# Ham3798/shielded-pool-pinocchio-solana

Hardware: AMD Instinct MI355X
Metric: Groth16 proofs/sec (higher is better)
Workload: dtype u32x8 (254-bit Montgomery integers); 1 GPU; audit_circuit (RLWE, const-PK; scripts/generate_audit.py:246-465), batch of 2048 independent proofs per GPU per step, every row a distinct witness; circuit=audit, n_constraints=29178, n_wires=35432, domain=32768, batch_per_gpu=2048, n_distinct_witnesses=2048, table_bytes=226725433344, parallelism=independent proofs x1, pk_bytes=9850060

## Files before the change

### include/spp.h

```cpp
#ifndef SPP_H
#define SPP_H
#include <stddef.h>
#include <stdint.h>
#ifdef __cplusplus
extern "C" {
#endif

#define SPP_OK 0
#define SPP_ERR_BAD_INPUT (-1)
#define SPP_ERR_NO_DEVICE (-2)
#define SPP_ERR_IO (-3)
#define SPP_ERR_UNSAT (-4)
#define SPP_ERR_HIP (-5)
#define SPP_ERR_NOT_IMPLEMENTED (-6)
#define SPP_ERR_FORMAT (-7)

#define SPP_CIRCUIT_WITHDRAW 1
#define SPP_CIRCUIT_AUDIT 2
#define SPP_CIRCUIT_WITHDRAW_REFSHAPE 3
#define SPP_CIRCUIT_WITHDRAW_DEPTH20 4

#define SPP_PROOF_LEN 388
#define SPP_WITHDRAW_PW_LEN 172
#define SPP_AUDIT_PW_LEN 76
// ... 36 lines not shown
int spp_circuit_msm_windows(const spp_circuit* c, uint32_t bits[7]);
int spp_circuit_msm_table_rows(const spp_circuit* c, uint32_t rows[7]);
int spp_circuit_small_rows(const spp_circuit* c, uint32_t out[2]);
uint64_t spp_circuit_table_bytes(const spp_circuit* c);

int spp_prove_batch(spp_circuit* c, size_t count, const uint8_t* inputs, const uint8_t* rs, uint8_t* proofs, uint8_t* pws,
                    int32_t* status);
int spp_prove_batch_device(spp_circuit* c, size_t count, const void* d_inputs, const void* d_rs, void* d_proofs, void* d_pws,
                           void* d_status);
int spp_sync(spp_circuit* c);
int spp_commitment_challenge(spp_circuit* c, size_t count, const uint8_t* inputs, uint8_t* challenges);
int spp_last_timings(spp_circuit* c, float ms[9]);
int spp_timings(spp_circuit* c, int which, float ms[9]);

int spp_msm_kernel_ms(spp_circuit* c, int which, float ms[7]);
int spp_set_serial(spp_circuit* c, int on);

int spp_prove_withdraw(spp_circuit* c, const spp_withdraw_inputs* in, const uint8_t rs_seed[64], uint8_t proof[SPP_PROOF_LEN],
                       uint8_t pw[SPP_WITHDRAW_PW_LEN]);

int spp_verify(const uint8_t* vk, size_t vk_len, const uint8_t* proof, size_t proof_len, const uint8_t* pw, size_t pw_len, int* ok);

int spp_debug_witness(spp_circuit* c, uint8_t* out, size_t n_wires);

#define SPP_ARITH_FR 0x000u
#define SPP_ARITH_FQ 0x100u
int spp_debug_arith(spp_ctx* ctx, uint32_t selector, uint32_t arg, size_t n, const uint32_t* in, size_t in_words, uint32_t* out,
                    size_t out_words);

int spp_rlwe_witness_batch(spp_ctx* ctx, const uint32_t* pk_a, const uint32_t* pk_b, size_t count, const int8_t* r, const int8_t* e1,
                           const int8_t* e2, const uint8_t* msg, uint32_t* c0, uint32_t* c1, int32_t* k0, int32_t* k1,
                           uint8_t* packed_be);
int spp_rlwe_witness_batch_device(spp_ctx* ctx, const void* d_pk_a, const void* d_pk_b, size_t count, const void* d_r, const void* d_e1,
                                  const void* d_e2, const void* d_msg, void* d_c0, void* d_c1, void* d_k0, void* d_k1,
                                  void* d_packed_be);
int spp_ctx_sync(spp_ctx* ctx);
int spp_poseidon_hash_batch(spp_ctx* ctx, size_t count, int arity, const uint8_t* in, uint8_t* out);
int spp_merkle_root_batch(spp_ctx* ctx, size_t count, uint32_t depth, const uint8_t* leaves, const uint64_t* indices,
                          const uint8_t* siblings, uint8_t* roots);
int spp_merkle_build(spp_ctx* ctx, size_t n_leaves, uint32_t depth, const uint8_t* leaves, size_t n_queries,
                     const uint64_t* query_indices, uint8_t* siblings_out, uint8_t* root_out);
typedef struct spp_merkle_tree spp_merkle_tree;
int spp_merkle_tree_new(spp_ctx* ctx, uint32_t depth, spp_merkle_tree** out);
void spp_merkle_tree_free(spp_merkle_tree* t);
uint64_t spp_merkle_tree_size(const spp_merkle_tree* t);
int spp_merkle_tree_insert(spp_merkle_tree* t, size_t count, const uint8_t* leaves, uint64_t* first_index);
// ... 121 lines not shown
```

### shielded-pool-pinocchio-solana_amd/csrc/kernels.hpp

```cpp
#pragma once
#include <hip/hip_runtime.h>
#include <stdint.h>
#include "bn254.hpp"
#include "f29.hpp"
#include "msm_plan.hpp"
#include "msm_ragged.hpp"
#include "rlwe_ntt.hpp"

namespace spp {

struct DevSparse {
  const uint32_t* rowptr;
  const uint32_t* wire;
  const uint32_t* coeff;
  const uint32_t* lit;
};
static constexpr uint32_t COEFF_ONE = 0x80000000u;
static constexpr uint32_t COEFF_MINUS_ONE = 0x40000000u;
static constexpr uint32_t COEFF_MASK = 0x3fffffffu;

struct HashConsts {
  const Fr* pos3_rc;  const Fr* pos3_mds;
  const Fr* pos5_rc;  const Fr* pos5_mds;
  const Fr* p2_rc;    const Fr* p2_mu;
// ... 115 lines not shown
                       int32_t* ok, uint32_t* list, uint32_t* n_list, uint32_t* stats);
void launch_verify_rlc_list(hipStream_t st, const VerifyKeyDev* vk, const RlcKeyDev* rk, const uint8_t* proofs, const uint8_t* pws, uint32_t pw_len,
                            uint32_t max_count, const uint32_t* in_list, const uint32_t* n_in, const RlcSeed& seed, uint32_t group, W256* ws,
                            uint32_t* live, int32_t* ok, uint32_t* list, uint32_t* n_list, uint32_t* stats);
struct PoolSet;
struct PoolState;
void launch_pool_screen_audit(hipStream_t st, const PoolSet& audits, uint64_t salt, const uint8_t* pws, uint32_t count, int32_t* prov, uint32_t* list,
                              uint32_t* n_list);
void launch_pool_screen_withdraw(hipStream_t st, const PoolState* state, const PoolSet& audits, const PoolSet& nullifiers, uint64_t salt,
                                 const uint8_t* pws, const uint8_t* recipients, uint32_t count, int32_t* prov, uint64_t* amounts, uint32_t* list,
                                 uint32_t* n_list);
struct PoolLogView;
void launch_pool_screen_withdraw_log(hipStream_t st, const PoolLogView& view, const PoolSet& audits, const PoolSet& nullifiers, uint64_t salt,
                                     const uint8_t* pws, const uint8_t* recipients, const uint32_t* deposits_before, const uint32_t* audits_before,
                                     uint32_t count, int32_t* prov, uint64_t* amounts, uint32_t* list, uint32_t* n_list);
void launch_pool_scatter(hipStream_t st, const uint32_t* pos, uint32_t count, const int32_t* codes, int32_t* result, const uint64_t* amounts,
                         uint64_t* amounts_out);
void launch_pool_screen_import(hipStream_t st, const PoolSet& set, uint64_t salt, const uint8_t* keys, uint32_t count, int32_t* prov);
void launch_pool_contains(hipStream_t st, const PoolSet& set, uint64_t salt, const uint8_t* keys, uint32_t count, uint8_t* present);
void launch_pool_resolve(hipStream_t st, uint32_t* slots, uint32_t mask, uint64_t salt, const uint8_t* keys, uint32_t stride, uint32_t count,
                         const int32_t* prov, const int32_t* proof_ok, int32_t dup, int32_t* result);
void launch_pool_commit(hipStream_t st, const PoolSet& set, uint64_t salt, const uint8_t* keys, uint32_t stride, uint32_t count, const int32_t* result,
                        uint32_t* set_count);
void launch_spmv_check(hipStream_t st, DevCircuit dc, const Fr* W, Fr* abc, uint32_t n, uint32_t P, uint32_t* status, int16_t* small = nullptr);

void launch_ntt(hipStream_t st, Fr* data, uint32_t logn, uint32_t P, const Fr* tw, bool dif, uint32_t nbatch, size_t batch_stride,
                const Fr* post = nullptr);
void launch_scale_rows(hipStream_t st, Fr* data, const Fr* table, uint32_t n, uint32_t P, uint32_t nbatch, size_t batch_stride);
void launch_qap_pointwise(hipStream_t st, Fr* abc, uint32_t n, uint32_t P, Fr zinv);
void launch_qap_product(hipStream_t st, Fr* abc, uint32_t n, uint32_t P);

template <class F>
struct MsmWalk;
template <>
struct MsmWalk<Fq> {
  static constexpr uint32_t waves_per_simd = 3;
  static constexpr uint32_t rows_waves_per_simd = 2;
  static constexpr bool gather_ahead = false;
  static constexpr int product_form = F29_SCAN_SERIAL;
  static constexpr uint32_t occ(uint32_t Wt) { return Wt == 1 ? waves_per_simd : rows_waves_per_simd; }
};
template <>
struct MsmWalk<Fq2> {
  static constexpr uint32_t waves_per_simd = 2;
  static constexpr uint32_t rows_waves_per_simd = 1;
  static constexpr bool gather_ahead = false;
  static constexpr int product_form = F29_COLUMNS;
  static constexpr uint32_t occ(uint32_t Wt) { return Wt == 1 ? waves_per_simd : rows_waves_per_simd; }
};
template <class F>
void launch_build_table(hipStream_t st, const Affine<F>* bases, uint32_t N, uint32_t c, uint32_t Wt, uint32_t row0, uint32_t nrows,
                        Affine<F>* table, XYZZ<F>* tmp, F* tmp_pre, const MsmBlock* blocks = nullptr, uint32_t E = 0);
void launch_msm_digits(hipStream_t st, const uint32_t* rows, const Fr* scalars, int16_t* dig, uint32_t N, uint32_t P, uint32_t c);
template <class F>
void launch_msm_accumulate(hipStream_t st, const Affine<F>* table, const MsmBlock* blocks, const int16_t* dig, XYZZ<F>* partial, uint32_t N, uint32_t P,
                           uint32_t c, const MsmPlan& pl, hipEvent_t ev_start = nullptr, hipEvent_t ev_stop = nullptr, uint32_t* redo_count = nullptr);
template <class F>
void launch_msm_reduce(hipStream_t st, XYZZ<F>* partial, XYZZ<F>* out, uint32_t P, const MsmPlan& pl, uint32_t c, bool empty);
static constexpr uint32_t MSM_FOLD_SETS = 8;
static constexpr uint32_t MSM_FOLD_RADIX = 8;
template <class F>
struct MsmFoldSets {
  XYZZ<F>* partial[MSM_FOLD_SETS];
  XYZZ<F>* out[MSM_FOLD_SETS];
  uint32_t Sg[MSM_FOLD_SETS], R[MSM_FOLD_SETS], c[MSM_FOLD_SETS];
  uint32_t cur[MSM_FOLD_SETS], half[MSM_FOLD_SETS];
};
template <class F>
void launch_msm_reduce_multi(hipStream_t st, MsmFoldSets<F> fs, uint32_t nsets, uint32_t P);

void launch_g1_eval_basis(hipStream_t st, const G1Affine* pts, uint32_t n_pts, uint32_t logn, const Fr* scale, const Fr* tw_inv, G1XYZZ* work,
                          G1Affine* out);

void launch_g1_column_sums(hipStream_t st, const G1Affine* base, const uint32_t* row, const Fr* coeff, uint32_t nterms, const uint32_t* seg,
                           uint32_t nseg, G1XYZZ* work, G1Affine* out);

// ... 31 lines not shown
```

### shielded-pool-pinocchio-solana_amd/csrc/kernels_msm.hip

```cpp
#include "msm_table.hpp"

namespace spp {

template void launch_build_table<Fq>(hipStream_t, const Affine<Fq>*, uint32_t, uint32_t, uint32_t, uint32_t, uint32_t, Affine<Fq>*,
                                     XYZZ<Fq>*, Fq*, const MsmBlock*, uint32_t);
template void launch_msm_accumulate<Fq>(hipStream_t, const Affine<Fq>*, const MsmBlock*, const int16_t*, XYZZ<Fq>*, uint32_t, uint32_t, uint32_t,
                                        const MsmPlan&, hipEvent_t, hipEvent_t, uint32_t*);
template void launch_msm_reduce_multi<Fq>(hipStream_t, MsmFoldSets<Fq>, uint32_t, uint32_t);
template void launch_msm_reduce<Fq>(hipStream_t, XYZZ<Fq>*, XYZZ<Fq>*, uint32_t, const MsmPlan&, uint32_t, bool);
template void launch_fixed_base_mul<Fq>(hipStream_t, const Affine<Fq>*, uint32_t, const Fr*, uint32_t, Affine<Fq>*);

__global__ void __launch_bounds__(256) k_msm_digits(const uint32_t* __restrict__ rows, const Fr* __restrict__ scalars,
                                                    int16_t* __restrict__ dig, uint32_t N, uint32_t P, uint32_t Pp, uint32_t c, uint32_t W) {
  const uint64_t g = (uint64_t)blockIdx.x * blockDim.x + threadIdx.x;
  const uint32_t p = (uint32_t)(g % Pp), i = (uint32_t)(g / Pp);
  if (i >= N || p >= P) return;
  const Fr s = scalars[(size_t)rows[i] * P + p];
  uint32_t l[8];
  s.to_canonical(l);
  const bool neg = canonical_gt_half<FrParams>(l);
  if (neg) {
    uint32_t t[8];
    canonical_negate<FrParams>(l, t);
    SPP_UNROLL for (int k = 0; k < 8; k++) l[k] = t[k];
  }
  const uint32_t mask = (1u << c) - 1u, half = 1u << (c - 1);
  uint32_t carry = 0;
  int16_t* out = dig + (size_t)i * Pp + p;
  const size_t plane = (size_t)N * Pp;
#pragma unroll 1
  for (uint32_t j = 0; j < W; j++) {
    const uint32_t d = (l[0] & mask) + carry;
    SPP_UNROLL for (int k = 0; k < 7; k++) l[k] = (l[k] >> c) | (l[k + 1] << (32 - c));
    l[7] >>= c;
    const bool over = neg ? d > half : d >= half;
    int v = over ? (int)d - (int)(1u << c) : (int)d;
    carry = over ? 1u : 0u;
    if (neg) v = -v;
    out[(size_t)j * plane] = (int16_t)v;
  }
}
void launch_msm_digits(hipStream_t st, const uint32_t* rows, const Fr* scalars, int16_t* dig, uint32_t N, uint32_t P, uint32_t c) {
  if (N == 0 || P == 0) return;
  const uint32_t Pp = msm_padded_batch(P);
  const uint64_t lanes = (uint64_t)N * Pp;
  hipLaunchKernelGGL(k_msm_digits, dim3((uint32_t)((lanes + 255) / 256)), dim3(256), 0, st, rows, scalars, dig, N, P, Pp, c, msm_windows(c));
}

__device__ __forceinline__ XYZZ<Fq> g1_scalar_mul(const XYZZ<Fq>& pt, const Fr& k) {
  uint32_t c[8];
  k.to_canonical(c);
  XYZZ<Fq> acc = XYZZ<Fq>::infinity();
  if (pt.is_inf()) return acc;
#pragma unroll 1
  for (int w = 7; w >= 0; w--) {
    const uint32_t word = w == 0 ? c[0] : w == 1 ? c[1] : w == 2 ? c[2] : w == 3 ? c[3] : w == 4 ? c[4] : w == 5 ? c[5] : w == 6 ? c[6] : c[7];
#pragma unroll 1
    for (int bit = 31; bit >= 0; bit--) {
      acc.dbl_inplace();
      if ((word >> bit) & 1) acc.add(pt);
    }
  }
  return acc;
}
__global__ void __launch_bounds__(64) k_g1_dft_load(const G1Affine* __restrict__ pts, uint32_t n_pts, const Fr* __restrict__ scale,
                                                    G1XYZZ* __restrict__ x, uint32_t n) {
  const uint32_t j = blockIdx.x * blockDim.x + threadIdx.x;
  if (j >= n) return;
  x[j] = j < n_pts ? g1_scalar_mul(G1XYZZ::from_affine(pts[j]), scale[j]) : G1XYZZ::infinity();
// ... 51 lines not shown
```

### shielded-pool-pinocchio-solana_amd/csrc/kernels_solve.hip

```cpp
#include "kernels.hpp"
#include "circuit.hpp"
#include "poseidon29.hpp"
#include "poseidon2.hpp"
#include "gnark_hints.hpp"
#include "sha256.hpp"

namespace spp {

__device__ __forceinline__ Fr dev_row_dot(const DevSparse& m, const Fr* __restrict__ coeffs, uint32_t k, uint32_t k_end_skip,
                                           const Fr* __restrict__ W, uint32_t P, uint32_t p, uint32_t first = 0, uint32_t step = 1) {
  Fr acc = Fr::zero();
  const uint32_t b = m.rowptr[k] + first, e = m.rowptr[k + 1] - k_end_skip;
  for (uint32_t t = b; t < e; t += step) {
    const uint32_t ci = m.coeff[t];
    Fr w = W[(size_t)m.wire[t] * P + p];
    if (ci & COEFF_ONE) acc = acc + w;
    else if (ci & COEFF_MINUS_ONE) acc = acc - w;
    else acc = acc + coeffs[ci & COEFF_MASK] * w;
  }
  return acc;
}

__global__ void __launch_bounds__(256) k_load_inputs(const uint8_t* __restrict__ in_be, const uint8_t* __restrict__ rs_be,
                                                     Fr* __restrict__ W, uint32_t n_inputs, uint32_t n_wires, uint32_t P) {
// ... 754 lines not shown
  int v = pos ? (int)c[0] : neg ? -(int)n[0] : 0;
  const int lo = dc.sm_lo[s];
  if ((!pos && !neg) || v < lo || v > lo + 255) {
    atomicOr(&status[p], 1u);
    v = 0;
  }
  small[g] = (int16_t)v;
}
__global__ void __launch_bounds__(256) k_spmv_small_rows(DevCircuit dc, const int16_t* __restrict__ small, const Fr* __restrict__ W,
                                                         Fr* __restrict__ abc, uint32_t n, uint32_t P) {
  const uint64_t g = (uint64_t)blockIdx.x * blockDim.x + threadIdx.x;
  if (g >= (uint64_t)dc.sm_nrows * P) return;
  const uint32_t p = (uint32_t)(g % P), r = (uint32_t)(g / P);
  const uint32_t b = dc.sm_rowptr[r], e = dc.sm_rowptr[r + 1];
  long long acc = 0;
  for (uint32_t t = b; t < e; t++) acc += (long long)dc.sm_coef[t] * (long long)small[(size_t)dc.sm_slot[t] * P + p];
  const uint32_t ro = dc.sm_row_out[r], mat = ro >> 30, k = ro & 0x3fffffffu;
  const Fr mag = Fr::from_u64((uint64_t)(acc < 0 ? -acc : acc));
  Fr v = acc < 0 ? mag.neg() : mag;
  for (uint32_t t = dc.sm_rest_ptr[r]; t < dc.sm_rest_ptr[r + 1]; t++) v = v + dc.coeffs[dc.sm_rest_coeff[t]] * W[(size_t)dc.sm_rest_wire[t] * P + p];
  abc[(size_t)mat * n * P + (size_t)k * P + p] = v;
}

__global__ void __launch_bounds__(256) k_spmv_check(DevCircuit dc, const Fr* __restrict__ W, Fr* __restrict__ abc, uint32_t n, uint32_t P,
                                                    uint32_t* __restrict__ status) {
  const uint64_t g = (uint64_t)blockIdx.x * blockDim.x + threadIdx.x;
  const uint64_t lanes = (uint64_t)(dc.n_runs + (n - dc.n_constraints)) * P;
  if (g >= lanes) return;
  const uint32_t p = (uint32_t)(g % P), r = (uint32_t)(g / P);
  const uint64_t total = (uint64_t)n * P;
  if (r >= dc.n_runs) {
    const uint64_t o = (uint64_t)(dc.n_constraints + (r - dc.n_runs)) * P + p;
    abc[o] = Fr::zero();
    abc[total + o] = Fr::zero();
    abc[2 * total + o] = Fr::zero();
    return;
  }
  const uint32_t k0 = dc.run_start[r], k1 = dc.run_start[r + 1];
  const uint8_t* __restrict__ rs = dc.row_small;
  const Fr b = (rs && (rs[k0] & 2)) ? abc[total + (uint64_t)k0 * P + p] : dev_row_dot_wide(dc.B, dc.coeffs, k0, W, P, p);
  bool bad = false;
  for (uint32_t k = k0; k < k1; k++) {
    const uint64_t o = (uint64_t)k * P + p;
    const uint32_t f = rs ? rs[k] : 0u;
    const Fr a = (f & 1) ? abc[o] : dev_row_dot_wide(dc.A, dc.coeffs, k, W, P, p);
    const Fr c = (f & 4) ? abc[2 * total + o] : dev_row_dot_wide(dc.C, dc.coeffs, k, W, P, p);
    bad |= (a * b != c);
    abc[o] = a;
    abc[total + o] = b;
    abc[2 * total + o] = c;
  }
  if (bad) atomicOr(&status[p], 1u);
}
static constexpr uint32_t LONG_G = 16;
__global__ void __launch_bounds__(1024) k_spmv_long_rows(DevCircuit dc, const Fr* __restrict__ W, Fr* __restrict__ abc, uint32_t n, uint32_t P) {
  __shared__ Fr part[LONG_G][64];
  const uint32_t lane = threadIdx.x & 63, sub = threadIdx.x >> 6, p = blockIdx.x * 64 + lane;
  const uint32_t code = dc.lg_rows[blockIdx.y], mi = code >> 30, k = code & 0x3fffffffu;
  const DevSparse& m = mi == 0 ? dc.A : mi == 1 ? dc.B : dc.C;
  part[sub][lane] = p < P ? dev_row_dot_wide(m, dc.coeffs, k, W, P, p, sub, LONG_G) : Fr::zero();
  __syncthreads();
  if (sub != 0 || p >= P) return;
  Fr acc = part[0][lane];
  SPP_UNROLL for (uint32_t q = 1; q < LONG_G; q++) acc = acc + part[q][lane];
  abc[(uint64_t)mi * n * P + (uint64_t)k * P + p] = acc;
}

static constexpr uint32_t SPMV_G = 16;
__device__ __forceinline__ Fr group_sum(Fr v) {
  SPP_UNROLL for (uint32_t off = SPMV_G / 2; off >= 1; off >>= 1) {
    Fr o;
    SPP_UNROLL for (int i = 0; i < 8; i++) o.l[i] = __shfl_xor(v.l[i], off);
    v = v + o;
  }
  return v;
}
__global__ void __launch_bounds__(256) k_spmv_check_rows(DevCircuit dc, const Fr* __restrict__ W, Fr* __restrict__ abc, uint32_t n, uint32_t P,
                                                         uint32_t* __restrict__ status) {
  const uint64_t g = (uint64_t)blockIdx.x * blockDim.x + threadIdx.x;
  const uint64_t total = (uint64_t)n * P;
  const uint64_t e = g / SPMV_G;
  const uint32_t sub = (uint32_t)(g % SPMV_G);
  const bool live = e < total;
  const uint32_t p = live ? (uint32_t)(e % P) : 0, k = live ? (uint32_t)(e / P) : dc.n_constraints;
  Fr a = Fr::zero(), b = Fr::zero(), c = Fr::zero();
  if (k < dc.n_constraints) {
    a = dev_row_dot_wide(dc.A, dc.coeffs, k, W, P, p, sub, SPMV_G);
    b = dev_row_dot_wide(dc.B, dc.coeffs, k, W, P, p, sub, SPMV_G);
    c = dev_row_dot_wide(dc.C, dc.coeffs, k, W, P, p, sub, SPMV_G);
  }
  a = group_sum(a);
  b = group_sum(b);
  c = group_sum(c);
  if (!live || sub != 0) return;
  if (a * b != c) atomicOr(&status[p], 1u);
  abc[e] = a;
  abc[total + e] = b;
  abc[2 * total + e] = c;
}
void launch_spmv_check(hipStream_t st, DevCircuit dc, const Fr* W, Fr* abc, uint32_t n, uint32_t P, uint32_t* status, int16_t* small) {
  if ((uint64_t)dc.n_runs * P < 65536 || (P <= 64 && dc.max_row_terms > 1024)) {
    const uint64_t lanes = (uint64_t)n * P * SPMV_G;
    hipLaunchKernelGGL(k_spmv_check_rows, dim3((uint32_t)((lanes + 255) / 256)), dim3(256), 0, st, dc, W, abc, n, P, status);
    return;
  }
  if (small && dc.sm_nrows) {
    const uint64_t l1 = (uint64_t)dc.sm_nslots * P, l2 = (uint64_t)dc.sm_nrows * P;
    hipLaunchKernelGGL(k_small_extract, dim3((uint32_t)((l1 + 255) / 256)), dim3(256), 0, st, dc, W, small, P, status);
    hipLaunchKernelGGL(k_spmv_small_rows, dim3((uint32_t)((l2 + 255) / 256)), dim3(256), 0, st, dc, small, W, abc, n, P);
  } else {
    dc.row_small = dc.row_long;
  }
  if (dc.lg_n) hipLaunchKernelGGL(k_spmv_long_rows, dim3((P + 63) / 64, dc.lg_n), dim3(1024), 0, st, dc, W, abc, n, P);
  const uint64_t lanes = (uint64_t)(dc.n_runs + (n - dc.n_constraints)) * P;
  hipLaunchKernelGGL(k_spmv_check, dim3((uint32_t)((lanes + 255) / 256)), dim3(256), 0, st, dc, W, abc, n, P, status);
}

}
```

### shielded-pool-pinocchio-solana_amd/csrc/spp_circuit.hpp

```cpp
#pragma once
#include "spp_internal.hpp"
#include "msm_classes.hpp"

template <class F>
struct MsmSet {
  uint32_t N = 0;
  Affine<F>* table = nullptr;
  uint32_t* rows = nullptr;
  bool from_h = false;
  uint32_t c = 0;
  uint32_t Wt = 0;
  MsmBlock* blocks = nullptr;
  bool narrow = false;
};
template <class F>
struct MsmBuf {
  XYZZ<F>* partial = nullptr;
  XYZZ<F>* out = nullptr;
  size_t partial_cap = 0;
  MsmPlan plan{};
};
struct Workspace {
  hipStream_t st = nullptr;
  hipStream_t st2 = nullptr;
// ... 18 lines not shown
  void* audit_scratch = nullptr;
  size_t audit_scratch_cap = 0;
  std::vector<void*> owned;
  hipEvent_t ev[8] = {};
  std::vector<std::pair<hipEvent_t, hipEvent_t>> msm_ev;
  size_t msm_ev_used = 0;
};

template <class F>
struct PendingTable {
  std::vector<Affine<F>> pts;
  Affine<F>* table;
  uint32_t c, Wt;
  MsmRagged layout;
  const MsmBlock* blocks;
};
struct SolveStep {
  enum Kind { SEQ, BATCH_DIV, COUNT8, COMMIT } kind;
  uint32_t a = 0, b = 0, c = 0;
  uint32_t ntracks = 0, tr_begin[COOP_TRACKS] = {}, tr_end[COOP_TRACKS] = {};
};
struct Switches {
  int h_mode = 2;
  bool no_coop = false;
  bool trace_items = false;
  bool one_track = false;
  bool no_level_stream = false;
  uint32_t coop_max_batch = 1024;
  bool no_side = false;
  int forced_depth = 0;
  bool no_split = false;
  bool ragged = true;
  MsmTuning msm;
};
static constexpr uint64_t SCALED_BLIND_MAX_SCALARS = 1500000;
inline uint32_t scaled_blind_max_batch(uint32_t n_a, uint32_t n_b1) {
  const uint64_t n = (uint64_t)n_a + n_b1;
  return n ? (uint32_t)std::max<uint64_t>(1, std::min<uint64_t>(1024, SCALED_BLIND_MAX_SCALARS / n)) : 1;
}
struct spp_circuit {
  spp_ctx* ctx = nullptr;
  std::vector<SolveStep> schedule;
  Circuit circ;
  DevCircuit dc{};
  uint32_t c_bits = 10, n = 0, logn = 0;
  uint32_t max_batch_div = SOLVE_SCRATCH_MIN_ROWS;
// ... 31 lines not shown
```

### shielded-pool-pinocchio-solana_amd/csrc/spp_load.cpp

```cpp
#include "spp_circuit.hpp"

static std::vector<PendingTable<Fq>>& pending(spp_circuit* c, Fq*) { return c->pending1; }
static std::vector<PendingTable<Fq2>>& pending(spp_circuit* c, Fq2*) { return c->pending2; }

static int upload_sparse(spp_circuit* c, const Circuit& circ, const Sparse& m, DevSparse* out) {
  std::vector<uint32_t> wire(m.terms.size()), coeff(m.terms.size()), lit(m.terms.size(), 0);
  Fr one = Fr::one(), mone = Fr::one().neg();
  std::vector<uint32_t> small(circ.coeffs.size(), 0);
  for (size_t ci = 0; ci < circ.coeffs.size(); ci++) {
    uint32_t v[8], nv[8];
    circ.coeffs[ci].to_canonical(v);
    bool hi0 = true;
    for (int k = 1; k < 8; k++) hi0 = hi0 && v[k] == 0;
    if (hi0 && v[0] != 0 && v[0] < (1u << 28)) { small[ci] = v[0]; continue; }
    circ.coeffs[ci].neg().to_canonical(nv);
    hi0 = true;
    for (int k = 1; k < 8; k++) hi0 = hi0 && nv[k] == 0;
    if (hi0 && nv[0] != 0 && nv[0] < (1u << 28)) small[ci] = nv[0] | 0x80000000u;
  }
  for (size_t i = 0; i < m.terms.size(); i++) {
    wire[i] = m.terms[i].wire;
    uint32_t ci = m.terms[i].coeff;
    uint32_t flag = 0;
    if (circ.coeffs[ci] == one) flag = COEFF_ONE;
// ... 196 lines not shown
  for (size_t i = 0; i < wires.size(); i++)
    if (wires[i] == wire) {
      pts[i] = host_add(pts[i], extra);
      return;
    }
  wires.push_back(wire);
  pts.push_back(extra);
}

struct LoadState {
  PkFile pk;
  uint32_t cw[7];
  WireClasses wc;
  bool flat[7] = {false, false, false, false, false, false, false};
  std::vector<uint32_t> z_w, xk_w;
  std::vector<G1Affine> z_p, xk_p;
};

static Switches read_switches() {
  Switches sw;
  const char* hm = getenv("SPP_H_MODE");
  sw.h_mode = hm ? atoi(hm) : (getenv("SPP_Z_COEFF") ? 0 : 2);
  if (sw.h_mode < 0 || sw.h_mode > 2) sw.h_mode = 2;
  sw.no_coop = getenv("SPP_NO_COOP") != nullptr;
  sw.trace_items = getenv("SPP_COOP_TRACE") != nullptr;
  sw.one_track = getenv("SPP_COOP_ONE_TRACK") != nullptr;
  sw.no_level_stream = getenv("SPP_NO_LEVEL_STREAM") != nullptr;
  if (const char* e = getenv("SPP_COOP_MAX")) sw.coop_max_batch = (uint32_t)atoi(e);
  sw.no_side = getenv("SPP_NO_SIDE") != nullptr;
  const char* de = getenv("SPP_DEPTH");
  const int depth = de ? atoi(de) : 0;
  sw.forced_depth = depth >= 1 && depth <= SPP_NWS ? depth : 0;
  sw.no_split = getenv("SPP_NO_SPLIT") != nullptr;
  const char* rg = getenv("SPP_RAGGED");
  sw.ragged = !(rg && rg[0] == '0');
  sw.msm = msm_tuning_from_env(getenv("SPP_MSM_WAVES"), getenv("SPP_MSM_WAVES_SMALL"));
  return sw;
}

static int plan_load_windows(const PkFile& pk, const WireClasses& wc, int window_bits, const uint32_t* forced_bits, uint32_t cw[7], bool flat[7]) {
  const double nset[7] = {(double)pk.A.size() + 2, (double)pk.B1.size() + 2, (double)pk.K.size() + 1, (double)pk.Z.size(),
                          (double)pk.CB.size(), (double)pk.CS.size(), (double)pk.B2.size() + 2};
  if (forced_bits) {
    for (int s = 0; s < 7; s++) {
      cw[s] = forced_bits[s];
      flat[s] = PLAN_WGT[s] != 0;
// ... 630 lines not shown
```

### shielded-pool-pinocchio-solana_amd/csrc/spp_prove.cpp

```cpp
#include "spp_circuit.hpp"

template <class T>
static int ws_alloc(Workspace& w, T** p, size_t count) {
  HIP_TRY(hipMalloc((void**)p, sizeof(T) * std::max<size_t>(count, 1)));
  w.owned.push_back((void*)*p);
  return 0;
}
template <class F>
static int ws_set(const spp_circuit* c, Workspace& w, const MsmSet<F>* s, MsmBuf<F>* b, size_t P) {
  b->partial_cap = msm_partial_cap(s->N, P, s->c, s->Wt, MsmWalk<F>::occ(s->Wt), c->sw.msm);
  int e;
  if ((e = ws_alloc(w, &b->partial, b->partial_cap))) return e;
  return ws_alloc(w, &b->out, P);
}
static int ensure_workspace(spp_circuit* c, Workspace& w, size_t P) {
  if (P <= w.cap) return 0;
  HIP_TRY(hipStreamSynchronize(w.st));
  free_workspace(w);
  int e;
  if ((e = ws_alloc(w, &w.W, (size_t)c->n_rows * P)) || (e = ws_alloc(w, &w.abc, (size_t)3 * c->n * P)) ||
      (e = ws_alloc(w, &w.scratch, (size_t)c->max_batch_div * P)) || (e = ws_alloc(w, &w.commit_affine, P)) ||
      (e = ws_alloc(w, &w.d_inputs, c->in_stride * P)) || (e = ws_alloc(w, &w.d_rs, 64 * P)) ||
      (e = ws_alloc(w, &w.d_proofs, (size_t)SPP_PROOF_LEN * P)) || (e = ws_alloc(w, &w.d_pws, c->pw_stride * P)) ||
      (e = ws_alloc(w, &w.d_status, P)) || (e = ws_alloc(w, &w.counters, 256 * P)))
// ... 4 lines not shown
    return e;
  {
    const size_t Ps = std::min<size_t>(P, scaled_blind_max_batch(c->A.N, c->B1.N));
    if ((e = ws_set(c, w, &c->A, &w.sA, Ps)) || (e = ws_set(c, w, &c->B1, &w.rB, Ps)) || (e = ws_alloc(w, &w.Ws, (size_t)c->n_rows * Ps)) ||
        (e = ws_alloc(w, &w.Wr, (size_t)c->n_rows * Ps)))
      return e;
  }
  {
    size_t d1 = 0;
    for (const MsmSet<Fq>* s : {&c->A, &c->B1, &c->K, &c->Z, &c->CB, &c->CS}) d1 = std::max(d1, msm_digit_elems(s->N, (uint32_t)P, s->c));
    w.dig1_cap = d1;
    w.dig2_cap = msm_digit_elems(c->B2.N, (uint32_t)P, c->B2.c);
    if ((e = ws_alloc(w, &w.dig1, w.dig1_cap)) || (e = ws_alloc(w, &w.dig2, w.dig2_cap))) return e;
    if (c->dc.sm_nrows && (e = ws_alloc(w, &w.small, (size_t)c->dc.sm_nslots * P))) return e;
  }
  w.cap = P;
  return 0;
}

static int16_t* ws_dig(Workspace& w, Fq*) { return w.dig1; }
static int16_t* ws_dig(Workspace& w, Fq2*) { return w.dig2; }
template <class F>
static void run_msm(spp_circuit* c, Workspace& w, const MsmSet<F>& s, MsmBuf<F>& b, uint32_t P, bool timed, hipStream_t st_override = nullptr,
                    std::pair<hipEvent_t, hipEvent_t>* ev_override = nullptr, bool fold = true, const Fr* scal_override = nullptr) {
  hipStream_t st = st_override ? st_override : w.st;
  const Fr* scal = scal_override ? scal_override : s.from_h ? w.abc : w.W;
  MsmPlan pl = msm_plan(s.N, P, s.c, s.Wt, MsmWalk<F>::occ(s.Wt), c->sw.msm);
  pl.fit(P, b.partial_cap);
  b.plan = pl;
  std::pair<hipEvent_t, hipEvent_t>* ev = nullptr;
  if (timed && w.msm_ev_used < w.msm_ev.size()) ev = &w.msm_ev[w.msm_ev_used++];
  if (ev_override) ev = ev_override;
  int16_t* dig = ws_dig(w, (F*)nullptr);
  launch_msm_digits(st, s.rows, scal, dig, s.N, P, s.c);
  launch_msm_accumulate<F>(st, s.table, s.blocks, dig, b.partial, s.N, P, s.c, pl, ev ? ev->first : nullptr, ev ? ev->second : nullptr);
  if (fold) launch_msm_reduce<F>(st, b.partial, b.out, P, pl, s.c, s.N == 0);
}

static int prove_on_device(spp_circuit* c, Workspace& w, uint32_t P, const uint8_t* d_inputs, const uint8_t* d_rs, uint8_t* d_proofs,
                           uint8_t* d_pws, uint32_t* d_status) {
  hipStream_t st = w.st;
  const Circuit& circ = c->circ;
  const uint32_t n = c->n;
  w.msm_ev_used = 0;
  w.last_P = P;
  const bool scaled_blind = P <= scaled_blind_max_batch(c->A.N, c->B1.N) && !c->sw.no_coop && !c->A.narrow && !c->B1.narrow;
  HIP_TRY(hipMemsetAsync(d_status, 0, sizeof(uint32_t) * P, st));
  hipEventRecord(w.ev[0], st);
  launch_load_inputs(st, d_inputs, d_rs, w.W, circ.n_inputs(), circ.n_wires, P);
  hipEventRecord(w.ev_in, st);
  for (const SolveStep& s : c->schedule) {
    switch (s.kind) {
      case SolveStep::SEQ:
        if (P <= c->sw.coop_max_batch && !c->sw.no_coop && c->sw.trace_items) {
          for (uint32_t t = 0; t < s.ntracks; t++)
            for (uint32_t it = s.tr_begin[t]; it < s.tr_end[t]; it++) {
              CoopTracks one{};
// ... 9 lines not shown
              CoopTracks one{};
              one.n = 1; one.begin[0] = s.tr_begin[t]; one.end[0] = s.tr_end[t];
              launch_solve_coop(st, c->dc, c->coop, w.W, w.scratch, one, P);
            }
          } else launch_solve_coop(st, c->dc, c->coop, w.W, w.scratch, tr, P);
        }
        else launch_solve(st, c->dc, w.W, w.scratch, s.a, s.b, P);
        break;
      case SolveStep::BATCH_DIV: launch_batch_div(st, c->dc, w.W, w.scratch, s.a, s.b, P); break;
      case SolveStep::COUNT8: launch_count8(st, c->dc, w.W, w.counters, s.a, s.b, s.c, P); break;
      case SolveStep::COMMIT:
        run_msm(c, w, c->CB, w.CB, P, true);
        launch_challenge(st, w.CB.out, w.W, circ.challenge_wire, P, w.commit_affine, d_status);
        break;
    }
  }
  hipEventRecord(w.ev[1], st);
  hipEventRecord(w.ev_w, st);
  hipStream_t side = (w.st2 != w.st && w.own_st2p && P > c->sw.coop_max_batch) ? w.own_st2p : w.st2;
  if (c->sw.no_side && P <= c->sw.coop_max_batch) side = st;
  hipStreamWaitEvent(side, w.ev_w, 0);
  run_msm(c, w, c->B2, w.B2, P, false, side, &w.g2_ev);
  hipEventRecord(w.ev_b2, side);
  launch_spmv_check(st, c->dc, w.W, w.abc, n, P, d_status, w.small);
  hipEventRecord(w.ev[2], st);
  const size_t bs = (size_t)n * P;
  const uint32_t nt = c->sw.h_mode == 2 ? 2 : 3;
  launch_ntt(st, w.abc, c->logn, P, c->tw_inv, true, nt, bs, c->coset_br);
  launch_ntt(st, w.abc, c->logn, P, c->tw_fwd, false, nt, bs);
  if (c->sw.h_mode == 2) launch_qap_product(st, w.abc, n, P);
  else launch_qap_pointwise(st, w.abc, n, P, c->zinv);
  if (c->sw.h_mode == 0) launch_ntt(st, w.abc, c->logn, P, c->tw_inv, true, 1, bs, c->coset_inv_br);
  hipEventRecord(w.ev[3], st);
  {
    MsmFoldSets<Fq> fs{};
    const MsmSet<Fq>* sets[7] = {&c->A, &c->B1, &c->K, &c->Z, &c->CS, &c->A, &c->B1};
    MsmBuf<Fq>* bufs[7] = {&w.A, &w.B1, &w.K, &w.Z, &w.CS, &w.sA, &w.rB};
    const Fr* scal[7] = {nullptr, nullptr, nullptr, nullptr, nullptr, w.Ws, w.Wr};
    const int nsets = scaled_blind ? 7 : 5;
    if (scaled_blind) launch_scale_witness(st, w.W, w.Ws, w.Wr, c->n_rows, c->row_r, c->row_s, P);
    for (int i = 0; i < nsets; i++) {
      run_msm(c, w, *sets[i], *bufs[i], P, i < 5, nullptr, nullptr, false, scal[i]);
      fs.partial[i] = bufs[i]->partial;
      fs.out[i] = bufs[i]->out;
      fs.Sg[i] = sets[i]->N ? bufs[i]->plan.Sg : 0;
      fs.R[i] = bufs[i]->plan.R;
      fs.c[i] = sets[i]->c;
    }
    launch_msm_reduce_multi<Fq>(st, fs, nsets, P);
  }
  hipEventRecord(w.ev[4], st);
  hipStreamWaitEvent(st, w.ev_b2, 0);
  hipEventRecord(w.ev[5], st);
  AssembleArgs a;
  a.mA = w.A.out; a.mB1 = w.B1.out; a.mB2 = w.B2.out; a.mK = w.K.out; a.mZ = w.Z.out; a.mPok = w.CS.out;
  a.commit_affine = w.commit_affine;
  a.W = w.W; a.row_r = c->row_r; a.row_s = c->row_s; a.n_public = circ.n_public;
  a.sAr = scaled_blind ? w.sA.out : nullptr;
  a.rBs1 = scaled_blind ? w.rB.out : nullptr;
  a.proofs = d_proofs; a.pws = d_pws; a.P = P;
  launch_assemble(st, a);
  hipEventRecord(w.ev[6], st);
  HIP_TRY(hipGetLastError());
  return SPP_OK;
}
// ... 382 lines not shown
  std::vector<uint8_t> buf(26 * 32, 0);
  auto put = [&](int i, const uint8_t* v) { memcpy(buf.data() + 32 * i, v, 32); };
  auto put64 = [&](int i, uint64_t v) { for (int k = 0; k < 8; k++) buf[32 * i + 31 - k] = (uint8_t)(v >> (8 * k)); };
  put(0, in->root); put(1, in->nullifier); put(2, in->recipient); put64(3, in->amount); put(4, in->wa_commitment);
  put(5, in->secret_key); put(6, in->owner_x); put(7, in->owner_y); put(8, in->randomness); put64(9, in->index);
  for (int i = 0; i < SPP_TREE_DEPTH; i++) put(10 + i, in->siblings[i]);
  int32_t st = 0;
  return spp_prove_batch(c, 1, buf.data(), rs_seed, proof, pw, &st);
}

extern "C" int spp_debug_witness(spp_circuit* c, uint8_t* out, size_t n_wires) {
  if (!c || !out) return fail(SPP_ERR_BAD_INPUT, "NULL argument");
  std::lock_guard<std::mutex> lk(c->ctx->mu);
  Workspace& w = c->ws[c->last_ws];
  if (w.cap == 0) return fail(SPP_ERR_BAD_INPUT, "no batch has been proved yet");
  HIP_TRY(hipSetDevice(c->ctx->device));
  HIP_TRY(hipStreamSynchronize(w.st));
  size_t P = w.last_P;
  std::vector<Fr> col(std::min<size_t>(n_wires, c->circ.n_wires));
  for (size_t i = 0; i < col.size(); i++) HIP_TRY(hipMemcpy(&col[i], w.W + i * P, sizeof(Fr), hipMemcpyDeviceToHost));
  for (size_t i = 0; i < col.size(); i++) col[i].to_bytes_be(out + 32 * i);
  return SPP_OK;
}
```

### shielded-pool-pinocchio-solana_amd/spp/prover.py

```python
import ctypes
import numpy as np
from .lib import load_library, check, SppError, PROOF_LEN, SPP_ERR_UNSAT, AUDIT_PW_LEN


def build_circuit(circuit_id, out_path, aux=None):
    L = load_library()
    n = ctypes.c_uint32(0)
    auxbuf = None
    if aux is not None:
        auxbuf = (ctypes.c_uint32 * len(aux))(*[int(v) for v in aux])
    check(L.spp_circuit_build(int(circuit_id), auxbuf, out_path.encode(), ctypes.byref(n)))
    return n.value


def verify(vk_bytes, proof_bytes, pw_bytes):
    L = load_library()
    ok = ctypes.c_int(0)
    check(L.spp_verify(vk_bytes, len(vk_bytes), proof_bytes, len(proof_bytes), pw_bytes, len(pw_bytes), ctypes.byref(ok)))
    return bool(ok.value)


def pairing_check_host(pairs):
    L = load_library()
    ok = ctypes.c_int(0)
# ... 293 lines not shown
    def prove_withdraw_notes_device(self, tree, count, d_notes, d_rs, d_proofs, d_pws, d_status):
        check(self.L.spp_prove_withdraw_notes_device(self.h, tree.h, count, d_notes, d_rs, d_proofs, d_pws, d_status))

    def sync(self):
        check(self.L.spp_sync(self.h))

    def last_timings(self, which=0):
        ms = (ctypes.c_float * 9)()
        check(self.L.spp_timings(self.h, int(which), ms))
        return list(ms)

    def msm_kernel_ms(self, which=0):
        ms = (ctypes.c_float * 7)()
        check(self.L.spp_msm_kernel_ms(self.h, int(which), ms))
        return list(ms)

    def set_serial(self, on):
        check(self.L.spp_set_serial(self.h, 1 if on else 0))

    def debug_witness(self):
        buf = ctypes.create_string_buffer(32 * self.n_wires)
        check(self.L.spp_debug_witness(self.h, ctypes.cast(buf, ctypes.c_void_p), self.n_wires))
        return [int.from_bytes(buf.raw[32 * i:32 * i + 32], "big") for i in range(self.n_wires)]
```

Before: 7399 proofs/s.

## Fuse QAP product into Z-MSM digit recoding and skip storing C evaluations

In product-form H mode, the spmv check no longer writes the C vector, and the separate qap_product kernel is removed. Instead, a new kernel computes a*b per Z-MSM row directly while recoding signed digits, so the product array is never materialised. This cuts one full-size Fr store in spmv, the product kernel's read/write pass, and a launch. In exchange the multiply is redone inside digit recoding, and only the Z rows' products are ever formed. It is enabled by default, with an env switch to disable it and a debug entry point for checking the fused digits against the old path.

```diff
diff --git a/include/spp.h b/include/spp.h
--- a/include/spp.h
+++ b/include/spp.h
@@ -82,6 +82,8 @@
 int spp_verify(const uint8_t* vk, size_t vk_len, const uint8_t* proof, size_t proof_len, const uint8_t* pw, size_t pw_len, int* ok);
 
 int spp_debug_witness(spp_circuit* c, uint8_t* out, size_t n_wires);
+
+int spp_debug_z_digits(spp_circuit* c, int fused, int16_t* out, size_t out_len, uint32_t dims[4]);
 
 #define SPP_ARITH_FR 0x000u
 #define SPP_ARITH_FQ 0x100u
diff --git a/profiles/fr_lean_trace_sums.py b/profiles/fr_lean_trace_sums.py
--- /dev/null
+++ b/profiles/fr_lean_trace_sums.py
@@ -0,0 +1,24 @@
+import csv
+import json
+import sys
+
+GROUPS = {"k_ntt_pass": "k_ntt_pass", "product": "k_qap_product", "digits": "k_msm_digits", "product_digits": "k_msm_product_digits",
+          "k_spmv_check": "k_spmv_check<", "k_spmv_small_rows": "k_spmv_small_rows", "k_spmv_long_rows": "k_spmv_long_rows"}
+
+
+def sums(path):
+    rows = list(csv.DictReader(open(path)))
+    def pick(sub):
+        return [r for r in rows if ("spp::" + sub) in r["Name"] or ("spp::" + sub.rstrip("<") + "(") in r["Name"]]
+    batches = sum(int(r["Calls"]) for r in pick("k_spmv_check<")) or 1
+    out = {"batches": batches}
+    for key, sub in GROUPS.items():
+        sel = pick(sub)
+        out[key] = {"launches_per_batch": sum(int(r["Calls"]) for r in sel) / batches,
+                    "ms_per_batch": round(sum(int(r["TotalDurationNs"]) for r in sel) / batches / 1e6, 3)}
+    out["fr_side_ms_per_batch"] = round(sum(v["ms_per_batch"] for k, v in out.items() if k != "batches"), 3)
+    return out
+
+
+if __name__ == "__main__":
+    print(json.dumps({"parent": sums(sys.argv[1]), "new": sums(sys.argv[2])}, indent=1))
diff --git a/shielded-pool-pinocchio-solana_amd/csrc/kernels.hpp b/shielded-pool-pinocchio-solana_amd/csrc/kernels.hpp
--- a/shielded-pool-pinocchio-solana_amd/csrc/kernels.hpp
+++ b/shielded-pool-pinocchio-solana_amd/csrc/kernels.hpp
@@ -161,7 +161,8 @@
                          const int32_t* prov, const int32_t* proof_ok, int32_t dup, int32_t* result);
 void launch_pool_commit(hipStream_t st, const PoolSet& set, uint64_t salt, const uint8_t* keys, uint32_t stride, uint32_t count, const int32_t* result,
                         uint32_t* set_count);
-void launch_spmv_check(hipStream_t st, DevCircuit dc, const Fr* W, Fr* abc, uint32_t n, uint32_t P, uint32_t* status, int16_t* small = nullptr);
+void launch_spmv_check(hipStream_t st, DevCircuit dc, const Fr* W, Fr* abc, uint32_t n, uint32_t P, uint32_t* status, int16_t* small = nullptr,
+                       bool store_c = true);
 
 void launch_ntt(hipStream_t st, Fr* data, uint32_t logn, uint32_t P, const Fr* tw, bool dif, uint32_t nbatch, size_t batch_stride,
                 const Fr* post = nullptr);
@@ -191,6 +192,7 @@
 void launch_build_table(hipStream_t st, const Affine<F>* bases, uint32_t N, uint32_t c, uint32_t Wt, uint32_t row0, uint32_t nrows,
                         Affine<F>* table, XYZZ<F>* tmp, F* tmp_pre, const MsmBlock* blocks = nullptr, uint32_t E = 0);
 void launch_msm_digits(hipStream_t st, const uint32_t* rows, const Fr* scalars, int16_t* dig, uint32_t N, uint32_t P, uint32_t c);
+void launch_msm_product_digits(hipStream_t st, const uint32_t* rows, const Fr* a, const Fr* b, int16_t* dig, uint32_t N, uint32_t P, uint32_t c);
 template <class F>
 void launch_msm_accumulate(hipStream_t st, const Affine<F>* table, const MsmBlock* blocks, const int16_t* dig, XYZZ<F>* partial, uint32_t N, uint32_t P,
                            uint32_t c, const MsmPlan& pl, hipEvent_t ev_start = nullptr, hipEvent_t ev_stop = nullptr, uint32_t* redo_count = nullptr);
diff --git a/shielded-pool-pinocchio-solana_amd/csrc/kernels_msm.hip b/shielded-pool-pinocchio-solana_amd/csrc/kernels_msm.hip
--- a/shielded-pool-pinocchio-solana_amd/csrc/kernels_msm.hip
+++ b/shielded-pool-pinocchio-solana_amd/csrc/kernels_msm.hip
@@ -1,4 +1,5 @@
 #include "msm_table.hpp"
+#include "msm_digits.hpp"
 
 namespace spp {
 
@@ -15,36 +16,27 @@
   const uint64_t g = (uint64_t)blockIdx.x * blockDim.x + threadIdx.x;
   const uint32_t p = (uint32_t)(g % Pp), i = (uint32_t)(g / Pp);
   if (i >= N || p >= P) return;
-  const Fr s = scalars[(size_t)rows[i] * P + p];
-  uint32_t l[8];
-  s.to_canonical(l);
-  const bool neg = canonical_gt_half<FrParams>(l);
-  if (neg) {
-    uint32_t t[8];
-    canonical_negate<FrParams>(l, t);
-    SPP_UNROLL for (int k = 0; k < 8; k++) l[k] = t[k];
-  }
-  const uint32_t mask = (1u << c) - 1u, half = 1u << (c - 1);
-  uint32_t carry = 0;
-  int16_t* out = dig + (size_t)i * Pp + p;
-  const size_t plane = (size_t)N * Pp;
-#pragma unroll 1
-  for (uint32_t j = 0; j < W; j++) {
-    const uint32_t d = (l[0] & mask) + carry;
-    SPP_UNROLL for (int k = 0; k < 7; k++) l[k] = (l[k] >> c) | (l[k + 1] << (32 - c));
-    l[7] >>= c;
-    const bool over = neg ? d > half : d >= half;
-    int v = over ? (int)d - (int)(1u << c) : (int)d;
-    carry = over ? 1u : 0u;
-    if (neg) v = -v;
-    out[(size_t)j * plane] = (int16_t)v;
-  }
+  msm_recode_scalar(scalars[(size_t)rows[i] * P + p], c, W, dig + (size_t)i * Pp + p, (size_t)N * Pp);
+}
+__global__ void __launch_bounds__(256) k_msm_product_digits(const uint32_t* __restrict__ rows, const Fr* __restrict__ a, const Fr* __restrict__ b,
+                                                            int16_t* __restrict__ dig, uint32_t N, uint32_t P, uint32_t Pp, uint32_t c, uint32_t W) {
+  const uint64_t g = (uint64_t)blockIdx.x * blockDim.x + threadIdx.x;
+  const uint32_t p = (uint32_t)(g % Pp), i = (uint32_t)(g / Pp);
+  if (i >= N || p >= P) return;
+  const size_t e = (size_t)rows[i] * P + p;
+  msm_recode_product(a[e], b[e], c, W, dig + (size_t)i * Pp + p, (size_t)N * Pp);
 }
 void launch_msm_digits(hipStream_t st, const uint32_t* rows, const Fr* scalars, int16_t* dig, uint32_t N, uint32_t P, uint32_t c) {
   if (N == 0 || P == 0) return;
   const uint32_t Pp = msm_padded_batch(P);
   const uint64_t lanes = (uint64_t)N * Pp;
   hipLaunchKernelGGL(k_msm_digits, dim3((uint32_t)((lanes + 255) / 256)), dim3(256), 0, st, rows, scalars, dig, N, P, Pp, c, msm_windows(c));
+}
+void launch_msm_product_digits(hipStream_t st, const uint32_t* rows, const Fr* a, const Fr* b, int16_t* dig, uint32_t N, uint32_t P, uint32_t c) {
+  if (N == 0 || P == 0) return;
+  const uint32_t Pp = msm_padded_batch(P);
+  const uint64_t lanes = (uint64_t)N * Pp;
+  hipLaunchKernelGGL(k_msm_product_digits, dim3((uint32_t)((lanes + 255) / 256)), dim3(256), 0, st, rows, a, b, dig, N, P, Pp, c, msm_windows(c));
 }
 
 __device__ __forceinline__ XYZZ<Fq> g1_scalar_mul(const XYZZ<Fq>& pt, const Fr& k) {
diff --git a/shielded-pool-pinocchio-solana_amd/csrc/kernels_solve.hip b/shielded-pool-pinocchio-solana_amd/csrc/kernels_solve.hip
--- a/shielded-pool-pinocchio-solana_amd/csrc/kernels_solve.hip
+++ b/shielded-pool-pinocchio-solana_amd/csrc/kernels_solve.hip
@@ -800,6 +800,7 @@
   abc[(size_t)mat * n * P + (size_t)k * P + p] = v;
 }
 
+template <bool STORE_C>
 __global__ void __launch_bounds__(256) k_spmv_check(DevCircuit dc, const Fr* __restrict__ W, Fr* __restrict__ abc, uint32_t n, uint32_t P,
                                                     uint32_t* __restrict__ status) {
   const uint64_t g = (uint64_t)blockIdx.x * blockDim.x + threadIdx.x;
@@ -811,7 +812,7 @@
     const uint64_t o = (uint64_t)(dc.n_constraints + (r - dc.n_runs)) * P + p;
     abc[o] = Fr::zero();
     abc[total + o] = Fr::zero();
-    abc[2 * total + o] = Fr::zero();
+    if (STORE_C) abc[2 * total + o] = Fr::zero();
     return;
   }
   const uint32_t k0 = dc.run_start[r], k1 = dc.run_start[r + 1];
@@ -826,7 +827,7 @@
     bad |= (a * b != c);
     abc[o] = a;
     abc[total + o] = b;
-    abc[2 * total + o] = c;
+    if (STORE_C) abc[2 * total + o] = c;
   }
   if (bad) atomicOr(&status[p], 1u);
 }
@@ -853,6 +854,7 @@
   }
   return v;
 }
+template <bool STORE_C>
 __global__ void __launch_bounds__(256) k_spmv_check_rows(DevCircuit dc, const Fr* __restrict__ W, Fr* __restrict__ abc, uint32_t n, uint32_t P,
                                                          uint32_t* __restrict__ status) {
   const uint64_t g = (uint64_t)blockIdx.x * blockDim.x + threadIdx.x;
@@ -874,12 +876,14 @@
   if (a * b != c) atomicOr(&status[p], 1u);
   abc[e] = a;
   abc[total + e] = b;
-  abc[2 * total + e] = c;
-}
-void launch_spmv_check(hipStream_t st, DevCircuit dc, const Fr* W, Fr* abc, uint32_t n, uint32_t P, uint32_t* status, int16_t* small) {
+  if (STORE_C) abc[2 * total + e] = c;
+}
+void launch_spmv_check(hipStream_t st, DevCircuit dc, const Fr* W, Fr* abc, uint32_t n, uint32_t P, uint32_t* status, int16_t* small,
+                       bool store_c) {
   if ((uint64_t)dc.n_runs * P < 65536 || (P <= 64 && dc.max_row_terms > 1024)) {
     const uint64_t lanes = (uint64_t)n * P * SPMV_G;
-    hipLaunchKernelGGL(k_spmv_check_rows, dim3((uint32_t)((lanes + 255) / 256)), dim3(256), 0, st, dc, W, abc, n, P, status);
+    if (store_c) hipLaunchKernelGGL(k_spmv_check_rows<true>, dim3((uint32_t)((lanes + 255) / 256)), dim3(256), 0, st, dc, W, abc, n, P, status);
+    else hipLaunchKernelGGL(k_spmv_check_rows<false>, dim3((uint32_t)((lanes + 255) / 256)), dim3(256), 0, st, dc, W, abc, n, P, status);
     return;
   }
   if (small && dc.sm_nrows) {
@@ -891,7 +895,8 @@
   }
   if (dc.lg_n) hipLaunchKernelGGL(k_spmv_long_rows, dim3((P + 63) / 64, dc.lg_n), dim3(1024), 0, st, dc, W, abc, n, P);
   const uint64_t lanes = (uint64_t)(dc.n_runs + (n - dc.n_constraints)) * P;
-  hipLaunchKernelGGL(k_spmv_check, dim3((uint32_t)((lanes + 255) / 256)), dim3(256), 0, st, dc, W, abc, n, P, status);
-}
-
-}
+  if (store_c) hipLaunchKernelGGL(k_spmv_check<true>, dim3((uint32_t)((lanes + 255) / 256)), dim3(256), 0, st, dc, W, abc, n, P, status);
+  else hipLaunchKernelGGL(k_spmv_check<false>, dim3((uint32_t)((lanes + 255) / 256)), dim3(256), 0, st, dc, W, abc, n, P, status);
+}
+
+}
diff --git a/shielded-pool-pinocchio-solana_amd/csrc/msm_digits.hpp b/shielded-pool-pinocchio-solana_amd/csrc/msm_digits.hpp
--- /dev/null
+++ b/shielded-pool-pinocchio-solana_amd/csrc/msm_digits.hpp
@@ -0,0 +1,33 @@
+#pragma once
+#include "bn254.hpp"
+
+namespace spp {
+
+SPP_HD void msm_recode_scalar(const Fr& s, uint32_t c, uint32_t W, int16_t* out, size_t plane) {
+  uint32_t l[8];
+  s.to_canonical(l);
+  const bool neg = canonical_gt_half<FrParams>(l);
+  if (neg) {
+    uint32_t t[8];
+    canonical_negate<FrParams>(l, t);
+    SPP_UNROLL for (int k = 0; k < 8; k++) l[k] = t[k];
+  }
+  const uint32_t mask = (1u << c) - 1u, half = 1u << (c - 1);
+  uint32_t carry = 0;
+#pragma unroll 1
+  for (uint32_t j = 0; j < W; j++) {
+    const uint32_t d = (l[0] & mask) + carry;
+    SPP_UNROLL for (int k = 0; k < 7; k++) l[k] = (l[k] >> c) | (l[k + 1] << (32 - c));
+    l[7] >>= c;
+    const bool over = neg ? d > half : d >= half;
+    int v = over ? (int)d - (int)(1u << c) : (int)d;
+    carry = over ? 1u : 0u;
+    if (neg) v = -v;
+    out[(size_t)j * plane] = (int16_t)v;
+  }
+}
+SPP_HD void msm_recode_product(const Fr& a, const Fr& b, uint32_t c, uint32_t W, int16_t* out, size_t plane) {
+  msm_recode_scalar(a * b, c, W, out, plane);
+}
+
+}
diff --git a/shielded-pool-pinocchio-solana_amd/csrc/spp_circuit.hpp b/shielded-pool-pinocchio-solana_amd/csrc/spp_circuit.hpp
--- a/shielded-pool-pinocchio-solana_amd/csrc/spp_circuit.hpp
+++ b/shielded-pool-pinocchio-solana_amd/csrc/spp_circuit.hpp
@@ -64,6 +64,7 @@
 };
 struct Switches {
   int h_mode = 2;
+  bool fr_lean = true;
   bool no_coop = false;
   bool trace_items = false;
   bool one_track = false;
diff --git a/shielded-pool-pinocchio-solana_amd/csrc/spp_load.cpp b/shielded-pool-pinocchio-solana_amd/csrc/spp_load.cpp
--- a/shielded-pool-pinocchio-solana_amd/csrc/spp_load.cpp
+++ b/shielded-pool-pinocchio-solana_amd/csrc/spp_load.cpp
@@ -242,6 +242,8 @@
   const char* hm = getenv("SPP_H_MODE");
   sw.h_mode = hm ? atoi(hm) : (getenv("SPP_Z_COEFF") ? 0 : 2);
   if (sw.h_mode < 0 || sw.h_mode > 2) sw.h_mode = 2;
+  const char* fl = getenv("SPP_FR_LEAN");
+  sw.fr_lean = !(fl && fl[0] == '0');
   sw.no_coop = getenv("SPP_NO_COOP") != nullptr;
   sw.trace_items = getenv("SPP_COOP_TRACE") != nullptr;
   sw.one_track = getenv("SPP_COOP_ONE_TRACK") != nullptr;
diff --git a/shielded-pool-pinocchio-solana_amd/csrc/spp_prove.cpp b/shielded-pool-pinocchio-solana_amd/csrc/spp_prove.cpp
--- a/shielded-pool-pinocchio-solana_amd/csrc/spp_prove.cpp
+++ b/shielded-pool-pinocchio-solana_amd/csrc/spp_prove.cpp
@@ -50,7 +50,8 @@
 static int16_t* ws_dig(Workspace& w, Fq2*) { return w.dig2; }
 template <class F>
 static void run_msm(spp_circuit* c, Workspace& w, const MsmSet<F>& s, MsmBuf<F>& b, uint32_t P, bool timed, hipStream_t st_override = nullptr,
-                    std::pair<hipEvent_t, hipEvent_t>* ev_override = nullptr, bool fold = true, const Fr* scal_override = nullptr) {
+                    std::pair<hipEvent_t, hipEvent_t>* ev_override = nullptr, bool fold = true, const Fr* scal_override = nullptr,
+                    bool digits_done = false) {
   hipStream_t st = st_override ? st_override : w.st;
   const Fr* scal = scal_override ? scal_override : s.from_h ? w.abc : w.W;
   MsmPlan pl = msm_plan(s.N, P, s.c, s.Wt, MsmWalk<F>::occ(s.Wt), c->sw.msm);
@@ -60,7 +61,7 @@
   if (timed && w.msm_ev_used < w.msm_ev.size()) ev = &w.msm_ev[w.msm_ev_used++];
   if (ev_override) ev = ev_override;
   int16_t* dig = ws_dig(w, (F*)nullptr);
-  launch_msm_digits(st, s.rows, scal, dig, s.N, P, s.c);
+  if (!digits_done) launch_msm_digits(st, s.rows, scal, dig, s.N, P, s.c);
   launch_msm_accumulate<F>(st, s.table, s.blocks, dig, b.partial, s.N, P, s.c, pl, ev ? ev->first : nullptr, ev ? ev->second : nullptr);
   if (fold) launch_msm_reduce<F>(st, b.partial, b.out, P, pl, s.c, s.N == 0);
 }
@@ -116,14 +117,17 @@
   hipStreamWaitEvent(side, w.ev_w, 0);
   run_msm(c, w, c->B2, w.B2, P, false, side, &w.g2_ev);
   hipEventRecord(w.ev_b2, side);
-  launch_spmv_check(st, c->dc, w.W, w.abc, n, P, d_status, w.small);
+  const bool lean = c->sw.h_mode == 2 && c->sw.fr_lean;
+  launch_spmv_check(st, c->dc, w.W, w.abc, n, P, d_status, w.small, !lean);
   hipEventRecord(w.ev[2], st);
   const size_t bs = (size_t)n * P;
   const uint32_t nt = c->sw.h_mode == 2 ? 2 : 3;
   launch_ntt(st, w.abc, c->logn, P, c->tw_inv, true, nt, bs, c->coset_br);
   launch_ntt(st, w.abc, c->logn, P, c->tw_fwd, false, nt, bs);
-  if (c->sw.h_mode == 2) launch_qap_product(st, w.abc, n, P);
-  else launch_qap_pointwise(st, w.abc, n, P, c->zinv);
+  if (!lean) {
+    if (c->sw.h_mode == 2) launch_qap_product(st, w.abc, n, P);
+    else launch_qap_pointwise(st, w.abc, n, P, c->zinv);
+  }
   if (c->sw.h_mode == 0) launch_ntt(st, w.abc, c->logn, P, c->tw_inv, true, 1, bs, c->coset_inv_br);
   hipEventRecord(w.ev[3], st);
   {
@@ -134,7 +138,9 @@
     const int nsets = scaled_blind ? 7 : 5;
     if (scaled_blind) launch_scale_witness(st, w.W, w.Ws, w.Wr, c->n_rows, c->row_r, c->row_s, P);
     for (int i = 0; i < nsets; i++) {
-      run_msm(c, w, *sets[i], *bufs[i], P, i < 5, nullptr, nullptr, false, scal[i]);
+      const bool z_lean = lean && sets[i] == &c->Z;
+      if (z_lean) launch_msm_product_digits(st, c->Z.rows, w.abc, w.abc + bs, w.dig1, c->Z.N, P, c->Z.c);
+      run_msm(c, w, *sets[i], *bufs[i], P, i < 5, nullptr, nullptr, false, scal[i], z_lean);
       fs.partial[i] = bufs[i]->partial;
       fs.out[i] = bufs[i]->out;
       fs.Sg[i] = sets[i]->N ? bufs[i]->plan.Sg : 0;
@@ -563,3 +569,33 @@
   for (size_t i = 0; i < col.size(); i++) col[i].to_bytes_be(out + 32 * i);
   return SPP_OK;
 }
+
+extern "C" int spp_debug_z_digits(spp_circuit* c, int fused, int16_t* out, size_t out_len, uint32_t dims[4]) {
+  if (!c || !dims) return fail(SPP_ERR_BAD_INPUT, "NULL argument");
+  if (c->sw.h_mode != 2 || !c->sw.fr_lean) return fail(SPP_ERR_BAD_INPUT, "the circuit was not loaded in the product form without the product store");
+  std::lock_guard<std::mutex> lk(c->ctx->mu);
+  Workspace& w = c->ws[c->last_ws];
+  if (w.cap == 0 || w.last_P == 0) return fail(SPP_ERR_BAD_INPUT, "no batch has been proved yet");
+  HIP_TRY(hipSetDevice(c->ctx->device));
+  HIP_TRY(hipStreamSynchronize(w.st));
+  const uint32_t P = (uint32_t)w.last_P, N = c->Z.N, Pp = msm_padded_batch(P), W = msm_windows(c->Z.c);
+  dims[0] = W; dims[1] = N; dims[2] = Pp; dims[3] = P;
+  if (!out) return SPP_OK;
+  const size_t elems = msm_digit_elems(N, P, c->Z.c), bs = (size_t)c->n * P;
+  if (out_len != elems) return fail(SPP_ERR_BAD_INPUT, "out holds %zu digits, the planes have %zu", out_len, elems);
+  DevBuf d_dig, d_ab;
+  HIP_TRY(d_dig.alloc(sizeof(int16_t) * std::max<size_t>(elems, 1)));
+  HIP_TRY(hipMemsetAsync(d_dig.p, 0, sizeof(int16_t) * elems, w.st));
+  if (fused) {
+    launch_msm_product_digits(w.st, c->Z.rows, w.abc, w.abc + bs, d_dig.as<int16_t>(), N, P, c->Z.c);
+  } else {
+    HIP_TRY(d_ab.alloc(sizeof(Fr) * 2 * bs));
+    HIP_TRY(hipMemcpyAsync(d_ab.p, w.abc, sizeof(Fr) * 2 * bs, hipMemcpyDeviceToDevice, w.st));
+    launch_qap_product(w.st, d_ab.as<Fr>(), c->n, P);
+    launch_msm_digits(w.st, c->Z.rows, d_ab.as<Fr>(), d_dig.as<int16_t>(), N, P, c->Z.c);
+  }
+  HIP_TRY(hipGetLastError());
+  HIP_TRY(hipStreamSynchronize(w.st));
+  HIP_TRY(hipMemcpy(out, d_dig.p, sizeof(int16_t) * elems, hipMemcpyDeviceToHost));
+  return SPP_OK;
+}
diff --git a/shielded-pool-pinocchio-solana_amd/spp/prover.py b/shielded-pool-pinocchio-solana_amd/spp/prover.py
--- a/shielded-pool-pinocchio-solana_amd/spp/prover.py
+++ b/shielded-pool-pinocchio-solana_amd/spp/prover.py
@@ -339,3 +339,12 @@
         buf = ctypes.create_string_buffer(32 * self.n_wires)
         check(self.L.spp_debug_witness(self.h, ctypes.cast(buf, ctypes.c_void_p), self.n_wires))
         return [int.from_bytes(buf.raw[32 * i:32 * i + 32], "big") for i in range(self.n_wires)]
+
+    def debug_z_digits(self, fused):
+        dims = (ctypes.c_uint32 * 4)()
+        self.L.spp_debug_z_digits.argtypes = [ctypes.c_void_p, ctypes.c_int, ctypes.c_void_p, ctypes.c_size_t, ctypes.POINTER(ctypes.c_uint32)]
+        check(self.L.spp_debug_z_digits(self.h, 1 if fused else 0, None, 0, dims))
+        n = dims[0] * dims[1] * dims[2]
+        buf = (ctypes.c_int16 * max(n, 1))()
+        check(self.L.spp_debug_z_digits(self.h, 1 if fused else 0, ctypes.cast(buf, ctypes.c_void_p), n, dims))
+        return tuple(dims), buf
```

Result: no change. 7414 proofs/s, median of 6 (+0.2%).
